# owkin/PyDESeq2

Measured on AMD Instinct MI355X. Metric: genes/sec end-to-end deseq2() (size factors->dispersion->IRLS->Wald), higher is better.
Workload: dtype f64

## Files before the change

### include/deseq_hip.h

```cpp
#ifndef DESEQ_HIP_H
#define DESEQ_HIP_H

#include <stddef.h>
#include <stdint.h>

#ifdef __cplusplus
extern "C" {
#endif

#define DSQ_ABI_VERSION 5
#define DSQ_MAX_P 128
#define DSQ_SHRINK_MAX_P 48
#define DSQ_BFGS_MAX_P 12

typedef struct dsq_ctx dsq_ctx;

enum dsq_status {
    DSQ_OK = 0,
    DSQ_ERR_HIP = -1,
    DSQ_ERR_ARG = -2,
    DSQ_ERR_RANGE = -3,
    DSQ_ERR_NOMEM = -4
};

// ... 138 lines not shown
                       int N, int G, int P, const double* d_alpha_hat, double min_disp, double max_disp,
                       double prior_disp_var, int cr_reg, int prior_reg, double* d_alpha, uint8_t* d_converged,
                       int32_t* d_nfev, double* d_nll_const, int const_mode, const dsq_cells* cells,
                       const double* d_coef, const double* d_sf, double min_mu);
int dsq_dev_alpha_mle3(dsq_ctx* ctx, const int32_t* d_y, const double* d_mu, int ldn, const double* d_Xt, int ldx,
                       int N, int G, int P, const double* d_alpha_hat, double min_disp, double max_disp,
                       double prior_disp_var, int cr_reg, int prior_reg, double* d_alpha, uint8_t* d_converged,
                       int32_t* d_nfev, double* d_nll_const, int const_mode, const dsq_cells* cells,
                       const double* d_coef, const double* d_sf, double min_mu, const int32_t* d_rows, int n_rows,
                       const int32_t* d_waves, int n_waves, const double* d_cell_mu);
typedef struct dsq_mix dsq_mix;
int dsq_mix_create(dsq_ctx* ctx, const double* design, int N, int P, dsq_mix** out);
void dsq_mix_destroy(dsq_mix* mix);
int dsq_mix_info(const dsq_mix* mix, int* n_slots, int* n_cells, int* n_continuous);
int dsq_mix_slots(const dsq_mix* mix, int32_t* h_slot_of);
int dsq_mix_bind(dsq_ctx* ctx, const uint16_t* d_ys, const uint8_t* d_big, const double* d_mu_slots);
int dsq_mix_bind2(dsq_ctx* ctx, const uint16_t* d_ys, const uint8_t* d_big, const double* d_mu_slots, int G);
int dsq_dev_mix_counts_to_slots(dsq_ctx* ctx, const int32_t* d_y, int ldn, int G, const dsq_mix* mix, uint16_t* d_ys,
                                uint8_t* d_big);
int dsq_dev_mix_mu_slots(dsq_ctx* ctx, const dsq_mix* mix, const double* d_beta, const double* d_sf, int G,
                         double* d_mu_slots);
int dsq_mix_takes_irls(const dsq_mix* mix, int full_rank);
int dsq_mix_launch_count(void);
int dsq_dev_alpha_mle4(dsq_ctx* ctx, const int32_t* d_y, const double* d_mu, int ldn, const double* d_Xt, int ldx,
                       int N, int G, int P, const double* d_alpha_hat, double min_disp, double max_disp,
                       double prior_disp_var, int cr_reg, int prior_reg, double* d_alpha, uint8_t* d_converged,
                       int32_t* d_nfev, double* d_nll_const, int const_mode, const dsq_cells* cells,
                       const double* d_coef, const double* d_sf, double min_mu, const int32_t* d_rows, int n_rows,
                       const int32_t* d_waves, int n_waves, const double* d_cell_mu, const dsq_mix* mix,
                       const double* d_beta);
int dsq_alpha_rows_eligible(int N, int P, int n_cells);
int dsq_alpha_needs_mu(int N, int P, int n_cells);
int dsq_dev_cell_mu(dsq_ctx* ctx, const double* d_beta, const dsq_cells* cells, int G, int P, double* d_cell_mu);
int dsq_dev_alpha_row_split(dsq_ctx* ctx, const int32_t* d_y, int ldn, int N, int G, int32_t* d_flags);
int dsq_dev_robust_disp(dsq_ctx* ctx, const int32_t* d_y, int ldn, const double* d_sf, const int32_t* d_cell_offsets,
                        const int32_t* d_cell_index, int n_cells, int whole, int max_cell, int N, int G,
                        double* d_robust_disp);
int dsq_dev_robust_disp2(dsq_ctx* ctx, const int32_t* d_y, int ldn, const double* d_sf, const int32_t* d_cell_offsets,
                         const int32_t* d_cell_index, int n_cells, int whole, int max_cell, int min_cell, int N, int G,
                         double* d_robust_disp);
int dsq_dev_lfc_fit(dsq_ctx* ctx, const int32_t* d_y, int ldn, const double* d_sf, const double* d_Xt,
                    const double* d_pinvXt, int ldx, int N, int G, int P, int full_rank, const double* d_disp,
                    double min_mu, double beta_tol, double min_beta, double max_beta, int maxiter, double* d_beta,
                    double* d_mu, double* d_hat, uint8_t* d_converged, int32_t* d_iters, const dsq_cells* cells,
                    const double* d_robust_disp, const uint8_t* d_flags, double cutoff, double* d_cooks,
                    uint8_t* d_any_all, uint8_t* d_any_use, uint8_t* d_any_use_nr, uint8_t* d_few_above,
// ... 144 lines not shown
```

### pydeseq2_amd/_lib.py

```python
from __future__ import annotations

import ctypes as C
import os

import numpy as np

_HERE = os.path.dirname(os.path.abspath(__file__))
LIB_PATH = os.environ.get("DSQ_LIB", os.path.join(_HERE, "libdeseq_hip.so"))

DSQ_MAX_P = 128
DSQ_SHRINK_MAX_P = 48
_DEBUG = bool(os.environ.get("DSQ_DEBUG"))
SAMPLE_MAJOR, GENE_MAJOR = 0, 1
I32, I64 = 0, 1
ALT = {None: 0, "greaterAbs": 1, "lessAbs": 2, "greater": 3, "less": 4}

c_void_p, c_int, c_double, c_size_t = C.c_void_p, C.c_int, C.c_double, C.c_size_t
_vp = c_void_p
HOOK_FN = C.CFUNCTYPE(None, c_void_p)


class DsqCells(C.Structure):

    _fields_ = [("d_cell_of", C.c_void_p), ("d_Xc", C.c_void_p), ("d_XX", C.c_void_p), ("n_cells", C.c_int)]
# ... 105 lines not shown
          c_double, c_int, _vp, _vp, _vp)
    proto("dsq_dev_lfc_shrink", _vp, _vp, c_int, _vp, _vp, c_int, c_int, c_int, c_int, _vp, c_double, c_double,
          c_int, _vp, _vp, _vp)
    proto("dsq_dev_lfc_shrink2", _vp, _vp, c_int, _vp, _vp, c_int, c_int, c_int, c_int, _vp, c_double, c_double,
          c_int, _vp, _vp, _vp, _vp)
    proto("dsq_dev_lfc_shrink3", _vp, _vp, c_int, _vp, _vp, c_int, c_int, c_int, c_int, _vp, c_double, c_double,
          c_int, _vp, _vp, _vp, _vp, c_int)
    proto("dsq_dev_padj_prepare", _vp, _vp, _vp, c_int, c_double, _vp, _vp, _vp, _vp, C.POINTER(c_int))
    proto("dsq_dev_padj_finish", _vp, _vp, _vp, _vp, c_int, c_int, c_int, _vp)
    proto("dsq_d2d", _vp, _vp, _vp, c_size_t)
    cells_p = C.POINTER(DsqCells)
    proto("dsq_dev_mom_lin_coef", _vp, _vp, c_int, _vp, _vp, _vp, c_int, c_int, c_int, c_int, c_double, c_double,
          c_double, _vp, _vp, _vp, _vp)
    proto("dsq_dev_alpha_mle2", _vp, _vp, _vp, c_int, _vp, c_int, c_int, c_int, c_int, _vp, c_double, c_double,
          c_double, c_int, c_int, _vp, _vp, _vp, _vp, c_int, cells_p, _vp, _vp, c_double)
    proto("dsq_dev_alpha_mle3", _vp, _vp, _vp, c_int, _vp, c_int, c_int, c_int, c_int, _vp, c_double, c_double,
          c_double, c_int, c_int, _vp, _vp, _vp, _vp, c_int, cells_p, _vp, _vp, c_double, _vp, c_int, _vp, c_int, _vp)
    proto("dsq_dev_alpha_mle4", _vp, _vp, _vp, c_int, _vp, c_int, c_int, c_int, c_int, _vp, c_double, c_double,
          c_double, c_int, c_int, _vp, _vp, _vp, _vp, c_int, cells_p, _vp, _vp, c_double, _vp, c_int, _vp, c_int, _vp,
          _vp, _vp)
    proto("dsq_mix_create", _vp, _vp, c_int, c_int, C.POINTER(_vp))
    proto("dsq_mix_destroy", _vp, res=None)
    proto("dsq_mix_launch_count")
    proto("dsq_mix_slots", _vp, _vp)
    proto("dsq_mix_takes_irls", _vp, c_int)
    proto("dsq_mix_info", _vp, C.POINTER(c_int), C.POINTER(c_int), C.POINTER(c_int))
    proto("dsq_alpha_rows_eligible", c_int, c_int, c_int)
    proto("dsq_alpha_needs_mu", c_int, c_int, c_int)
    proto("dsq_dev_cell_mu", _vp, _vp, cells_p, c_int, c_int, _vp)
    proto("dsq_dev_alpha_row_split", _vp, _vp, c_int, c_int, c_int, _vp)
    proto("dsq_dev_robust_disp", _vp, _vp, c_int, _vp, _vp, _vp, c_int, c_int, c_int, c_int, c_int, _vp)
    proto("dsq_dev_robust_disp2", _vp, _vp, c_int, _vp, _vp, _vp, c_int, c_int, c_int, c_int, c_int, c_int, _vp)
    proto("dsq_dev_lfc_fit", _vp, _vp, c_int, _vp, _vp, _vp, c_int, c_int, c_int, c_int, c_int, _vp, c_double,
          c_double, c_double, c_double, c_int, _vp, _vp, _vp, _vp, _vp, cells_p, _vp, _vp, c_double, _vp, _vp, _vp,
          _vp, _vp, _vp, _vp, c_double, c_int, _vp, _vp, _vp)
    proto("dsq_dev_lfc_fit2", _vp, _vp, c_int, _vp, _vp, _vp, c_int, c_int, c_int, c_int, c_int, _vp, c_double,
          c_double, c_double, c_double, c_int, _vp, _vp, _vp, _vp, _vp, cells_p, _vp, _vp, c_double, _vp, _vp, _vp,
          _vp, _vp, _vp, _vp, c_double, c_int, _vp, _vp, _vp, _vp, c_int)
    proto("dsq_dev_irls_layers", _vp, _vp, c_int, _vp, _vp, c_int, c_int, c_int, c_int, _vp, _vp, c_double, _vp, _vp)
    proto("dsq_side_begin", _vp)
    proto("dsq_side_end", _vp)
    proto("dsq_side_wait", _vp)
    proto("dsq_side_abort", _vp)
    proto("dsq_set_deferred", _vp, c_int)
    proto("dsq_lfc_fork_begin", _vp)
    proto("dsq_lfc_fork_end", _vp)
# ... 42 lines not shown
    return lib


EXPORTS = [
    "dsq_create", "dsq_destroy", "dsq_last_error", "dsq_device_info", "dsq_sync", "dsq_debug_pending_error", "dsq_timer_start",
    "dsq_timer_stop", "dsq_last_alpha_kernel", "dsq_malloc", "dsq_free", "dsq_memset", "dsq_h2d", "dsq_d2h", "dsq_h2d_2d",
    "dsq_d2h_2d", "dsq_inf_lin_reg_mu", "dsq_inf_irls", "dsq_inf_alpha_mle", "dsq_inf_wald_test",
    "dsq_inf_fit_rough_dispersions", "dsq_inf_fit_moments_dispersions", "dsq_dev_trend_loss_grad", "dsq_dev_trend_fit", "dsq_dev_prior_mad",
    "dsq_dev_counts_to_gene_major", "dsq_dev_f64_to_gene_major", "dsq_dev_logmeans",
    "dsq_dev_size_factors", "dsq_dev_mom", "dsq_dev_lin_mu", "dsq_dev_alpha_mle", "dsq_dev_irls",
    "dsq_dev_cooks", "dsq_dev_replace_outliers", "dsq_dev_wald", "dsq_dev_gather_rows_f64",
    "dsq_dev_gather_rows_i32", "dsq_comm_unique_id", "dsq_comm_init", "dsq_comm_destroy",
    "dsq_comm_allreduce_sum", "dsq_comm_allgather", "dsq_dev_sf_keys", "dsq_dev_sf_count", "dsq_dev_sf_init",
    "dsq_dev_sf_hist", "dsq_dev_sf_pick", "dsq_dev_sf_finish", "dsq_dev_trend_eval", "dsq_dev_trend_prior", "dsq_dev_select_dispersions",
    "dsq_dev_scatter_rows_f64", "dsq_d2d", "dsq_dev_mom_lin_mu", "dsq_dev_sf_keys_compact", "dsq_prior_mad_work_doubles", "dsq_size_factors_work_doubles", "dsq_dev_mom_raw", "dsq_dev_nll_const", "dsq_dev_nll_scaled", "dsq_dev_logmeans_poscounts", "dsq_dev_vst", "dsq_inf_lfc_shrink_nbinom_glm", "dsq_dev_lfc_shrink", "dsq_dev_lfc_shrink2", "dsq_dev_lfc_shrink3", "dsq_dev_padj_prepare", "dsq_dev_padj_finish", "dsq_host_alloc", "dsq_host_free", "dsq_d2h_async", "dsq_h2d_async",
    "dsq_dev_size_factors_new", "dsq_dev_mom_lin_coef", "dsq_dev_alpha_mle2", "dsq_dev_robust_disp", "dsq_dev_robust_disp2", "dsq_dev_lfc_fit", "dsq_dev_lfc_fit2", "dsq_dev_irls_layers",
    "dsq_side_begin", "dsq_side_end", "dsq_side_wait", "dsq_side_abort", "dsq_set_deferred", "dsq_irls_order_hint", "dsq_set_alpha_hook", "dsq_dev_alpha_mle3", "dsq_dev_alpha_mle4", "dsq_mix_create", "dsq_mix_destroy", "dsq_mix_info", "dsq_mix_slots", "dsq_mix_takes_irls", "dsq_dev_replace_outliers2", "dsq_mix_launch_count", "dsq_alpha_rows_eligible", "dsq_alpha_needs_mu", "dsq_dev_cell_mu", "dsq_dev_alpha_row_split",
    "dsq_upload_counts_i32", "dsq_inf_dispersion_trend_gamma_glm", "dsq_inf_grid_fit_alpha", "dsq_inf_grid_fit_beta",
    "dsq_inf_irls2", "dsq_inf_alpha_mle2", "dsq_inf_lfc_shrink_nbinom_glm2", "dsq_inf_fit_moments_dispersions2",
    "dsq_abi_version", "dsq_plugin_cache_config", "dsq_plugin_cache_clear", "dsq_plugin_cache_stats",
    "dsq_plugin_digest_host", "dsq_comm_info", "dsq_host_sync_count", "dsq_dev_pack2", "dsq_dev_unzip2",
    "dsq_mix_bind", "dsq_mix_bind2", "dsq_dev_mix_counts_to_slots", "dsq_dev_mix_mu_slots",
    "dsq_lfc_fork_begin", "dsq_lfc_fork_end", "dsq_lfc_set_part", "dsq_lfc_takes_parts", "dsq_dev_select_dispersions_part", "dsq_lfc_prepare", "dsq_alpha_set_late_flags",
    "dsq_dev_lrt", "dsq_dev_chisq_sf", "dsq_dev_wald_multi", "dsq_dev_rlog",
]


def ptr(a):
    if a is None:
        return None
    if isinstance(a, np.ndarray):
        return a.ctypes.data
    return a


class Context:

    def __init__(self, device: int = 0):
        self.lib = load()
        h = _vp()
        rc = self.lib.dsq_create(int(device), C.byref(h))
        if rc != 0 or not h.value:
            raise DsqError(
                f"dsq_create(device={device}) failed (rc={rc}): no usable MI355X / HIP runtime. "
                "pydeseq2_amd runs on the GPU only."
            )
        self.h = h
# ... 176 lines not shown
```

### pydeseq2_amd/csrc/dsq_capi_dev.hip

```cpp
#include "dsq_capi_internal.h"

extern "C" {

int dsq_dev_counts_to_gene_major(dsq_ctx* ctx, const void* d_src, int count_type, int layout, int N, int G,
                                 int32_t* d_dst, int ldn, int* h_bad) {
    DSQ_CHECK_ARG(ldn >= N, "ldn < N");
    int* d_bad = (int*)ctx->d_scratch;
    DSQ_HIP(hipMemsetAsync(d_bad, 0, sizeof(int), ctx->stream));
    DSQ_HIP(dsq::launch_transpose_counts(ctx->stream, d_src, count_type, layout, N, G, d_dst, ldn, d_bad));
    if (h_bad) {
        DSQ_HIP(hipMemcpyAsync(h_bad, d_bad, sizeof(int), hipMemcpyDeviceToHost, ctx->stream));
        DSQ_HIP(hipStreamSynchronize(ctx->stream));
    }
    return DSQ_OK;
}

int dsq_dev_f64_to_gene_major(dsq_ctx* ctx, const double* d_src, int layout, int N, int G, double* d_dst,
                              int ldn) {
    DSQ_HIP(dsq::launch_transpose_f64(ctx->stream, d_src, layout, N, G, d_dst, ldn));
    return DSQ_OK;
}

int dsq_dev_logmeans(dsq_ctx* ctx, const int32_t* d_y, int ldn, int N, int G, double* d_logmeans,
                     uint8_t* d_nonzero) {
// ... 355 lines not shown
    const int rc = dsq_mix_bind(ctx, d_ys, d_big, d_mu_slots);
    ctx->bind_G = (rc == DSQ_OK && G > 0) ? G : 0;
    return rc;
}
int dsq_dev_mix_counts_to_slots(dsq_ctx* ctx, const int32_t* d_y, int ldn, int G, const dsq_mix* mix, uint16_t* d_ys,
                                uint8_t* d_big) {
    DSQ_CHECK_ARG(mix != nullptr && d_y != nullptr && d_ys != nullptr && d_big != nullptr, "null argument");
    DSQ_HIP(dsq::launch_mix_counts_to_slots(ctx->stream, d_y, ldn, mix->d, G, d_ys, d_big));
    return DSQ_OK;
}
int dsq_dev_mix_mu_slots(dsq_ctx* ctx, const dsq_mix* mix, const double* d_beta, const double* d_sf, int G,
                         double* d_mu_slots) {
    DSQ_CHECK_ARG(mix != nullptr && d_beta != nullptr && d_sf != nullptr && d_mu_slots != nullptr, "null argument");
    DSQ_HIP(dsq::launch_mix_mu_slots(ctx->stream, d_beta, d_sf, mix->d, G, d_mu_slots));
    return DSQ_OK;
}

int dsq_mix_takes_irls(const dsq_mix* mix, int full_rank) {
    return (mix != nullptr && dsq::irls_takes_mix(&mix->d, full_rank)) ? 1 : 0;
}

int dsq_mix_launch_count(void) { return dsq::alpha_mix_launches(); }

int dsq_mix_info(const dsq_mix* mix, int* n_slots, int* n_cells, int* n_continuous) {
    if (mix == nullptr) return DSQ_ERR_ARG;
    if (n_slots) *n_slots = mix->d.Ns;
    if (n_cells) *n_cells = mix->d.C;
    if (n_continuous) *n_continuous = mix->d.Q;
    return DSQ_OK;
}

int dsq_alpha_needs_mu(int N, int P, int n_cells) { return dsq::alpha_needs_mu(N, P, n_cells) ? 1 : 0; }

int dsq_alpha_rows_eligible(int N, int P, int n_cells) {
    if (dsq::alpha_rows_eligible(N, P, n_cells, true, 1)) return 1;
    return dsq::alpha_rowsc_tail(N, P, n_cells) > 0 ? 2 : 0;
}

int dsq_dev_cell_mu(dsq_ctx* ctx, const double* d_beta, const dsq_cells* cells, int G, int P, double* d_cell_mu) {
    DSQ_CHECK_ARG(P >= 1 && P <= 12 && cells != nullptr && cells->n_cells > 0, "cells / P out of range");
    DSQ_HIP(dsq::launch_cell_mu(ctx->stream, d_beta, cells->d_Xc, cells->n_cells, G, P, d_cell_mu));
    return DSQ_OK;
}

int dsq_dev_alpha_row_split(dsq_ctx* ctx, const int32_t* d_y, int ldn, int N, int G, int32_t* d_flags) {
    DSQ_HIP(dsq::launch_count_big(ctx->stream, d_y, ldn, N, G, d_flags));
// ... 464 lines not shown
```

### pydeseq2_amd/csrc/dsq_irls.h

```cpp
#pragma once
#include "dsq_alpha.h"
#include "dsq_bfgs.h"
#include "dsq_lbfgsb.h"
#include "dsq_linalg.h"
#include "dsq_stats.h"
#include "dsq_wave.h"

#ifndef DSQ_IRLS_UNROLL
#define DSQ_IRLS_UNROLL 2
#endif
#define DSQ_PRAGMA_(x) _Pragma(#x)
#define DSQ_PRAGMA(x) DSQ_PRAGMA_(x)
#define DSQ_UNROLL2 DSQ_PRAGMA(unroll DSQ_IRLS_UNROLL)
#ifndef DSQ_IRLS_ROW_U
#define DSQ_IRLS_ROW_U 4
#endif

namespace dsq {

constexpr int kIrlsRowU = DSQ_IRLS_ROW_U;

struct LfcEpilogue {
    const uint8_t* flags = nullptr;
    double robust_disp = 0.0, cutoff = 0.0;
// ... 172 lines not shown
#pragma unroll
        for (int k = 0; k < NR; ++k)
            if (Wv::lane() + k * Wv::W < P) Wk.ent[T + Wv::lane() + k * Wv::W] = vr[k];
    }
    Wv::sync();
    if constexpr (LOADM) {
#pragma unroll
        for (int k = 0; k < T; ++k) M[k] = Wk.ent[k];
#pragma unroll
        for (int j = 0; j < P; ++j) r[j] = Wk.ent[T + j];
        Wv::sync();
    }
    S = Wv::sum(s);
}

template <int CS>
DSQ_HD double cell_select(int cell, const double (&v)[CS]) {
    double r = v[0];
#pragma unroll
    for (int c = 1; c < CS; ++c) r = (cell == c) ? v[c] : r;
    return r;
}

template <class Wv, int P, int CS>
DSQ_HD void irls_sweep_cs(const IrlsArgs& A, const double (&beta)[P], double a, double& S,
                          double (&M)[Tri<P>::N], double (&r)[P], double (&e_c)[CS]) {
    constexpr int T = Tri<P>::N;
    const CellDesign& D = *A.cells;
    const auto Xc_ = DSQ_AS_LDS(double, D.Xc);
    const auto XX_ = DSQ_AS_LDS(double, D.XX);
    double eta_c[CS], sw[CS], swz[CS];
#pragma unroll
    for (int c = 0; c < CS; ++c) {
        double eta = 0.0;
        if (c < D.C) {
#pragma unroll
            for (int j = 0; j < P; ++j) eta += Xc_[c * P + j] * beta[j];
        }
        eta_c[c] = Wv::uniform(eta);
        e_c[c] = Wv::uniform(exp(eta));
        sw[c] = 0.0;
        swz[c] = 0.0;
    }
    double s = 0.0;
    const double lmin = log(A.min_mu);
    DSQ_PHASE(3);
// ... 81 lines not shown
            const double h = w * cell_select<CS>(cell, q_c);
            if (H_out != nullptr) H_out[n] = h;
            if (want_cooks) {
                const double ck = acc.add(n, (double)A.y[n], mu_raw, h, E->flags[n]);
                if (E->cooks_row != nullptr) E->cooks_row[n] = ck;
            }
        }
        if (want_wald) {
            double wu = w;
            if (!have_w || Wv::any(!(mu_raw >= A.min_mu))) wu = mu_raw * frcp_g(1.0 + mu_raw * A.disp);
#pragma unroll
            for (int c = 0; c < CS; ++c) swu[c] += (cell == c) ? wu : 0.0;
        }
    }
    if (want_cooks) E->cooks = acc.finish(A.y, A.N);
    if (want_wald) {
        double Mw[T];
#pragma unroll
        for (int k = 0; k < T; ++k) Mw[k] = 0.0;
#pragma unroll
        for (int c = 0; c < CS; ++c) {
            if (c < D.C) {
                const double sc = Wv::sum(swu[c]);
#pragma unroll
                for (int k = 0; k < T; ++k) Mw[k] += XX_[c * T + k] * sc;
            }
        }
        E->wald = wald_from_M<P>(Mw, beta, E->ridge, E->contrast, E->lfc_null, E->alt);
    }
}

struct IrlsOut {
    int converged;
    int iters;
    int fallback;
};

template <class Wv, int P>
DSQ_HD void irls_init(const IrlsArgs& A, double a, double (&b0)[P], double& cst) {
#pragma unroll
    for (int j = 0; j < P; ++j) b0[j] = 0.0;
    double lga, dga_unused, tab_dl, tab_dd;
    lgamma_digamma<false, true>(a, lga, dga_unused);
    lgamma_digamma_diff<Wv, false>(Wv::lane(), a, lga, 0.0, tab_dl, tab_dd);
    double c = 0.0;
    for (int base = 0; base < A.N; base += Wv::W) {
// ... 267 lines not shown
            }
        }
    }
    for (; n < A.N; n += Wv::W) {
        const int cell = D.cell_of[n];
        const double wu = sample(n, cell, A.sf[n], Wk.tab[1][cell], Wk.acc[0][cell],
                                 want_cooks ? (double)A.y[n] : 0.0, want_cooks ? E->flags[n] : 0);
        if (want_wald) Wv::cell_add(&Wk.acc[1][cell], wu);
    }
    if (want_cooks) E->cooks = acc.finish(A.y, A.N);
    if (want_wald) {
        Wv::sync();
        for (int e = Wv::lane(); e < T; e += Wv::W) {
            Wk.ent[e] = cell_dot<T>(XX_ + e, Wk.acc[1], D.C);
        }
        Wv::sync();
        double Mw[T];
#pragma unroll
        for (int k = 0; k < T; ++k) Mw[k] = Wk.ent[k];
        E->wald = wald_from_M<P>(Mw, beta, E->ridge, E->contrast, E->lfc_null, E->alt);
    }
}

template <class Wv, int P, int CELL = 0>
DSQ_HD IrlsOut irls_gene(const IrlsArgs& A, double (&beta)[P], double* mu_out, double* H_out,
                         LfcEpilogue* E = nullptr) {
    constexpr int T = Tri<P>::N;
    IrlsOut out;
    out.converged = 1; out.iters = 0; out.fallback = 0;
    const double a = 1.0 / A.disp;
    double cst;
    DSQ_PHASE(1);
    if constexpr (CELL == 1 && Wv::W == 16) {
        if (A.pinvc != nullptr) irls_init_cell<Wv, P>(A, a, beta, cst);
        else irls_init<Wv, P>(A, a, beta, cst);
    } else {
        irls_init<Wv, P>(A, a, beta, cst);
    }
    const double nlogterm = A.N * a * log(A.disp);
    double M[T], r[P], S;
    constexpr int CS = CELL == 3 ? 2 : kSmallCells;
    double e_c[CS];
    constexpr bool kRowSolve = CELL == 1 && Wv::W == 16;
    auto sweep = [&]() {
        DSQ_PHASE(2);
        if constexpr (CELL == 1) irls_sweep_cell<Wv, P, !kRowSolve>(A, beta, a, S, M, r);
        else if constexpr (CELL >= 2) irls_sweep_cs<Wv, P, CS>(A, beta, a, S, M, r, e_c);
        else irls_sweep<Wv, P>(A, beta, a, S, M, r);
        DSQ_PHASE(5);
    };
    sweep();
    double dev = 1000.0, ratio = 1.0;
    int i = 0;
    while (ratio > A.beta_tol) {
        double bh[P];
        if constexpr (kRowSolve) {
            typedef DSQ_LDS_STRUCT(CellWork<P>) LdsWork;
            DSQ_PHASE(7);
            row_chol_solve<Wv, P>(((LdsWork*)A.cell_ws)->ent, 1e-6, bh);
            Wv::sync();
        } else {
            double Hm[T];
#pragma unroll
            for (int k = 0; k < T; ++k) Hm[k] = M[k];
#pragma unroll
            for (int j = 0; j < P; ++j) Hm[tri(j, j)] += 1e-6;
            DSQ_PHASE(7);
            chol<P>(Hm);
            DSQ_PHASE(8);
#pragma unroll
            for (int j = 0; j < P; ++j) bh[j] = r[j];
            chol_solve<P>(Hm, bh);
        }
        DSQ_PHASE(5);
        i += 1;
        bool bad = (i >= A.maxiter);
#pragma unroll
        for (int j = 0; j < P; ++j) bad = bad || (fabs(bh[j]) > A.max_beta);
        if (bad) {
            out.fallback = 1; out.converged = 0; out.iters = i;
            return out;
        }
#pragma unroll
        for (int j = 0; j < P; ++j) beta[j] = bh[j];
        sweep();
        const double old = dev;
        dev = -2.0 * (nlogterm - cst + S);
        ratio = fabs(dev - old) / (fabs(dev) + 0.1);
    }
    out.iters = i;
    DSQ_PHASE(6);
    if constexpr (kRowSolve) {
        typedef DSQ_LDS_STRUCT(CellWork<P>) LdsWork;
        LdsWork& Wk = *(LdsWork*)A.cell_ws;
#pragma unroll
        for (int k = 0; k < T; ++k) M[k] = Wk.ent[k];
        Wv::sync();
    }
    if constexpr (CELL == 1) irls_finish_cell<Wv, P>(A, beta, M, mu_out, H_out, E);
    else if constexpr (CELL >= 2) irls_finish_cs<Wv, P, CS>(A, beta, M, e_c, mu_out, H_out, E);
    else irls_finish<Wv, P>(A, beta, M, mu_out, H_out, E);
    return out;
}

template <int P>
struct IrlsRescueWork {
    union {
        LbfgsbWork<P> lb;
        BfgsWork<P> bf;
    };
    double x[P], l[P], u[P];
    int nbd[P];
};

template <class Wv>
DSQ_HD void grid_fit_beta2(const IrlsArgs& A, double a, double cst, double (&beta)[2],
                           int grid_length = 60) {
    auto loss = [&](double bx, double by) {
        double s = 0.0;
        DSQ_UNROLL2
    for (int n = Wv::lane(); n < A.N; n += Wv::W) {
            const double yv = (double)A.y[n];
            const double eta = A.Xt[n] * bx + A.Xt[A.ldx + n] * by;
// ... 91 lines not shown
```

### pydeseq2_amd/csrc/dsq_k_irls.hip

```cpp
#include <type_traits>

#include "dsq_dispatch.h"
#include "dsq_irls.h"
#include "dsq_launch.h"

namespace dsq {

#if defined(DSQ_PHASE_TIMING)
__device__ unsigned long long g_phase_total_irls[16];
#endif

#ifndef DSQ_IRLS_WAVES_P2
#define DSQ_IRLS_WAVES_P2 4
#endif
constexpr int irls_min_waves(int p) { return p <= 2 ? DSQ_IRLS_WAVES_P2 : (p <= 5 ? 1 : 2); }

template <int P, int CELL>
__global__ __launch_bounds__(kBlock, CELL == 1 ? cell_min_waves(P) : irls_min_waves(P)) void k_irls(const int32_t* __restrict__ y, int ldn,
                                                 const double* __restrict__ sf, const double* __restrict__ lsf,
                                                 const double* __restrict__ Xt,
                                                 const double* __restrict__ pinvXt, int ldx, int N,
                                                 int G, int full_rank, const double* __restrict__ disp,
                                                 double min_mu, double beta_tol, double min_beta,
                                                 double max_beta, int maxiter, double* __restrict__ beta,
                                                 double* __restrict__ mu, double* __restrict__ hat,
                                                 uint8_t* __restrict__ conv, int32_t* __restrict__ iters,
                                                 int32_t* __restrict__ fb_count,
                                                 int32_t* __restrict__ fb_list, IrlsExtras ex, int stage) {
    __shared__ typename std::conditional<CELL == 1, CellWork<P>, char>::type cellw[kWavesPerBlock];
    extern __shared__ __attribute__((aligned(16))) double irls_lds[];
    const int w = threadIdx.x >> 6;
    const int g = blockIdx.x * kWavesPerBlock + w;
    if (ex.part != nullptr) {
        bool any = false;
#pragma unroll
        for (int k = 0; k < kWavesPerBlock; ++k) {
            const int gk = blockIdx.x * kWavesPerBlock + k;
            any = any || (gk < G && ex.part[gk] == (uint8_t)ex.part_want);
        }
        if (!any) return;
// ... 26 lines not shown
        sf = s_sf;
        if (lsf != nullptr) lsf = s_lsf;
        if (CELL) ex.cells.cell_of = s_cell;
        yrow = s_y;
    }
    __syncthreads();
    if (g >= G) return;
    if (ex.part != nullptr && ex.part[g] != (uint8_t)ex.part_want) return;
#if defined(DSQ_PHASE_TIMING)
    if ((threadIdx.x & 63) == 0) {
        for (int k = 0; k < kPhases; ++k) g_ph_acc[w][k] = 0;
        g_ph_last[w] = clock64();
        g_ph_cur[w] = 0;
    }
#endif
    IrlsArgs A;
    A.y = yrow; A.sf = sf; A.lsf = lsf; A.Xt = Xt; A.pinvXt = pinvXt; A.ldx = ldx; A.N = N;
    A.disp = disp[g]; A.min_mu = min_mu; A.beta_tol = beta_tol; A.min_beta = min_beta;
    A.max_beta = max_beta; A.maxiter = maxiter; A.full_rank = full_rank != 0;
    if (CELL) { A.cells = &ex.cells; A.cell_ws = CELL == 1 ? (void*)&cellw[w] : nullptr; }
    LfcEpilogue E;
    epilogue_begin(E, ex, g, ldn);
    double b[P];
    const IrlsOut o = irls_gene<DeviceWave, P, CELL>(A, b, mu ? mu + (size_t)g * ldn : nullptr,
                                                     hat ? hat + (size_t)g * ldn : nullptr, &E);
    if ((threadIdx.x & 63) == 0) {
#pragma unroll
        for (int j = 0; j < P; ++j) beta[(size_t)g * P + j] = b[j];
        conv[g] = (uint8_t)o.converged;
        if (iters != nullptr) iters[g] = o.iters;
        if (o.fallback) fb_list[atomicAdd(fb_count, 1)] = g;
        else epilogue_store(E, ex, g);
    }
#if defined(DSQ_PHASE_TIMING)
    DSQ_PHASE(0);
    if ((threadIdx.x & 63) == 0)
        for (int k = 0; k < kPhases; ++k) atomicAdd(&g_phase_total_irls[k], (unsigned long long)g_ph_acc[w][k]);
#endif
}

constexpr int kRowGenes = kBlock / 16;
template <int P>
__global__ __launch_bounds__(kBlock, 2) void k_irls_row(const int32_t* __restrict__ y, int ldn,
                                                        const double* __restrict__ sf, const double* __restrict__ lsf,
                                                        const double* __restrict__ Xt,
                                                        const double* __restrict__ pinvXt, int ldx, int N, int G,
                                                        int full_rank, const double* __restrict__ disp, double min_mu,
                                                        double beta_tol, double min_beta, double max_beta, int maxiter,
// ... 249 lines not shown
                                          Xt, ldx, N, G, disp, beta, min_mu, mu, hat))
    return hipGetLastError();
}

constexpr int kRowMinP = 3;
static bool row_wave_enabled() {
    static const bool v = getenv("DSQ_NO_ROW_WAVE") == nullptr;
    return v;
}
static int row_min_p() {
    static const int v = getenv("DSQ_ROW_MIN_P") ? atoi(getenv("DSQ_ROW_MIN_P")) : 5;
    return v;
}
static size_t row_lds_bytes(int C, int P, int N) {
    const int npad = (N + 15) & ~15;
    return (size_t)C * (P * (P + 1) / 2 + 2 * P) * sizeof(double) + (size_t)npad * 20 + (size_t)kMaxCells * 4;
}

static int irls_row_min_genes() {
    const char* e = getenv("DSQ_IRLS_ROW_MIN_G");
    return e ? atoi(e) : 1024;
}

bool irls_takes_parts(int N, int P_, int n_cells, const MixDesign* mix, int full_rank) {
    (void)N;
    if (mix != nullptr && irls_takes_mix(mix, full_rank)) return true;
    return !(P_ > DSQ_REG_MAX_P || (P_ >= wide_min_p() && (n_cells == 0 || wide_with_cells())));
}

bool irls_takes_rows(int N, int P_, int n_cells) {
    if (P_ > DSQ_REG_MAX_P || (P_ >= wide_min_p() && (n_cells == 0 || wide_with_cells()))) return false;
    return n_cells > kSmallCells && P_ >= kRowMinP && P_ >= row_min_p() && row_wave_enabled() &&
           row_lds_bytes(n_cells, P_, N) <= 40 * 1024;
}

#define DSQ_MIXI_DECL(Q_)                                                                                             \
    bool irls_mix_fits_q##Q_(int Ns, int P);                                                                          \
    void irls_mix_grid_q##Q_(int Ns, int P, int G, int* blocks, int* nw);                                             \
    hipError_t launch_irls_mix_q##Q_(hipStream_t, const int32_t*, int, const uint16_t*, const uint8_t*, const MixDesign&, \
                                     const double*, int, int32_t*, const double*, double, double, double, int, double*, \
                                     double*, double*, uint8_t*, int32_t*, int32_t*, int32_t*, const IrlsExtras&, void*, \
                                     size_t);
DSQ_MIXI_DECL(1)
DSQ_MIXI_DECL(2)
DSQ_MIXI_DECL(3)
#undef DSQ_MIXI_DECL
// ... 38 lines not shown
                       const double* Xt,
                       const double* pinvXt, int ldx, int N, int G, int P_, int full_rank,
                       const double* disp, double min_mu, double beta_tol, double min_beta,
                       double max_beta, int maxiter, double* beta, double* mu, double* hat,
                       uint8_t* conv, int32_t* iters, int32_t* fb_count, int32_t* fb_list,
                       const IrlsExtras* extras) {
    if (G <= 0) return hipSuccess;
    IrlsExtras ex{};
    if (extras != nullptr) ex = *extras;
    if (ex.mix != nullptr && ex.mix_work != nullptr && ex.mix_queue != nullptr && ex.mix_ys != nullptr &&
        ex.mix_big != nullptr && irls_takes_mix(ex.mix, full_rank))
        return launch_irls_mix(st, y, ldn, *ex.mix, sf, G, ex.mix_queue, disp, min_mu, beta_tol, max_beta, maxiter, beta,
                               mu, hat, conv, iters, fb_count, fb_list, ex, ex.mix_work, ex.mix_work_bytes);
    if (P_ > DSQ_REG_MAX_P || (P_ >= wide_min_p() && (ex.cells.C == 0 || wide_with_cells()))) {
        if (ex.cells.C > 0 && ex.cells.C <= kSmallCells) ex.cells = CellDesign{};
        return launch_wide_irls(st, y, ldn, sf, lsf, Xt, pinvXt, ldx, N, G, P_, full_rank, disp, min_mu, beta_tol,
                                min_beta, max_beta, maxiter, beta, mu, hat, conv, iters, fb_count, fb_list, &ex);
    }
    const dim3 grid(genes_to_blocks(G)), block(kBlock);
    const int npad = (N + 15) & ~15;
    const size_t stage_bytes = (size_t)npad * (16 + 4 + 4 * kWavesPerBlock);
    static const bool allow_stage = getenv("DSQ_IRLS_NO_STAGE") == nullptr;
    if (ex.cells.C > 0 && ex.cells.C <= kSmallCells && P_ <= 4) {
        DSQ_DISPATCH_P(P_, {
            if constexpr (P <= 4) {
                const size_t tables = (size_t)ex.cells.C * (Tri<P>::N + P) * sizeof(double);
                const int stage = allow_stage && tables + stage_bytes <= 48 * 1024;
                if (ex.cells.C <= 2 && P <= 2)
                    hipLaunchKernelGGL((k_irls<(P <= 2 ? P : 1), 3>), grid, block, tables + (stage ? stage_bytes : 0),
                                       st, y, ldn, sf, lsf, Xt, pinvXt, ldx, N, G, full_rank, disp, min_mu, beta_tol,
                                       min_beta, max_beta, maxiter, beta, mu, hat, conv, iters, fb_count, fb_list, ex,
                                       stage);
                else
                    hipLaunchKernelGGL((k_irls<P, 2>), grid, block, tables + (stage ? stage_bytes : 0), st, y, ldn,
                                       sf, lsf, Xt, pinvXt, ldx, N, G, full_rank, disp, min_mu, beta_tol, min_beta,
                                       max_beta, maxiter, beta, mu, hat, conv, iters, fb_count, fb_list, ex, stage);
            }
        })
    } else if (irls_takes_rows(N, P_, ex.cells.C) && G >= irls_row_min_genes()) {
        const dim3 grid_r((G + kRowGenes - 1) / kRowGenes);
        DSQ_DISPATCH_P(P_, {
            if constexpr (P >= kRowMinP)
                hipLaunchKernelGGL((k_irls_row<P>), grid_r, block, row_lds_bytes(ex.cells.C, P, N), st, y, ldn, sf, lsf,
                                   Xt, pinvXt, ldx, N, G, full_rank, disp, min_mu, beta_tol, min_beta, max_beta, maxiter,
                                   beta, mu, hat, conv, iters, fb_count, fb_list, ex);
        })
    } else if (ex.cells.C > kSmallCells && P_ >= 3) {
        DSQ_DISPATCH_P(P_, {
            if constexpr (P >= 3) {
                const size_t tables = (size_t)ex.cells.C * (Tri<P>::N + P) * sizeof(double);
                const int stage = allow_stage && tables + stage_bytes <= 48 * 1024;
                hipLaunchKernelGGL((k_irls<P, 1>), grid, block, tables + (stage ? stage_bytes : 0), st, y, ldn, sf,
                                   lsf, Xt, pinvXt, ldx, N, G, full_rank, disp, min_mu, beta_tol, min_beta, max_beta,
                                   maxiter, beta, mu, hat, conv, iters, fb_count, fb_list, ex, stage);
            }
        })
    } else {
        const int stage = allow_stage && stage_bytes <= 48 * 1024;
        DSQ_DISPATCH_P(P_, hipLaunchKernelGGL((k_irls<P, 0>), grid, block, stage ? stage_bytes : 0, st, y, ldn, sf,
// ... 68 lines not shown
```

### pydeseq2_amd/csrc/dsq_launch.h

```cpp
#pragma once
#include <hip/hip_runtime.h>

#include <cstdint>

#include "../../include/deseq_hip.h"
#include "dsq_irls.h"
#include "dsq_linalg.h"
#include "dsq_mix.h"

namespace dsq {

constexpr int kWavesPerBlock = 4;
constexpr int kBlock = 64 * kWavesPerBlock;

inline int genes_to_blocks(int G) { return (G + kWavesPerBlock - 1) / kWavesPerBlock; }

inline int current_device_cus() {
    static int cache[64] = {0};
    int dev = 0;
    if (hipGetDevice(&dev) != hipSuccess) return 0;
    if (dev >= 0 && dev < 64 && cache[dev] > 0) return cache[dev];
    hipDeviceProp_t prop;
    if (hipGetDeviceProperties(&prop, dev) != hipSuccess) return 0;
    if (dev >= 0 && dev < 64) cache[dev] = prop.multiProcessorCount;
// ... 74 lines not shown
size_t alpha_resume_bytes(int G);
constexpr int kRowTail = 512;
bool alpha_rows_eligible(int N, int P, int n_cells, bool has_coef, int cr_reg);
hipError_t launch_alpha_rows(hipStream_t st, const int32_t* y, int ldn, int N, const int32_t* list, int n_list,
                             int32_t* queue, const double* coef, const double* sf, const CellDesign& cells, int P,
                             double min_mu, const double* alpha_hat, double min_disp, double max_disp, double prior_var,
                             int cr_reg, int prior_reg, double* alpha, uint8_t* conv, int32_t* nfev, int32_t* grid_count,
                             int32_t* grid_list, double* nll_const, int const_mode, int eval_cap, void* park_state,
                             int32_t* park_count, int32_t* park_list);
hipError_t launch_count_big(hipStream_t st, const int32_t* y, int ldn, int N, int G, int32_t* out);
int alpha_rowsc_tail(int N, int P, int n_cells);
hipError_t launch_alpha_rows_c(hipStream_t st, const int32_t* y, int ldn, int N, const int32_t* list, int n_list,
                               int32_t* queue, const double* coef, const double* cell_mu, const double* sf,
                               const CellDesign& cells, int P, double min_mu, const double* alpha_hat, double min_disp,
                               double max_disp, double prior_var, int prior_reg, double* alpha, uint8_t* conv,
                               int32_t* nfev, int32_t* grid_count, int32_t* grid_list, double* nll_const,
                               int const_mode, int eval_cap, void* park_state, int32_t* park_count,
                               int32_t* park_list);
hipError_t launch_cell_mu(hipStream_t st, const double* beta, const double* Xc, int C, int G, int P, double* cell_mu);
hipError_t launch_mu_from_cells(hipStream_t st, const double* cell_mu, int C, const double* sf, const int32_t* cell_of,
                                int N, const int32_t* list, int n_list, double* dst, int ldn, int32_t* idx_out,
                                const int32_t* n_dev = nullptr);
bool alpha_mix_enabled();
int alpha_mix_launches();
bool alpha_mix_fits(const MixDesign& D);
hipError_t launch_alpha_mix(hipStream_t st, const uint16_t* ys, const double* mu_s, const MixDesign& D, const int32_t* list,
                            int n_list, const int32_t* n_dev, int32_t* queue, const double* alpha_hat, double min_disp,
                            double max_disp, double prior_var, int prior_reg, double* alpha, uint8_t* conv, int32_t* nfev,
                            int32_t* grid_count, int32_t* grid_list, double* nll_const, int const_mode, int eval_cap,
                            int resume, void* park_state, int32_t* park_count, int32_t* park_list);
hipError_t launch_mu_from_beta(hipStream_t st, const double* beta, const double* sf, const double* Xt, int ldx, int N,
                               int P, const int32_t* list, int n_list, double* dst, int ldn, int32_t* idx_out,
                               const int32_t* n_dev = nullptr);
bool alpha_wg_eligible(int N);
hipError_t launch_alpha_wg(hipStream_t st, const int32_t* y, int ldn, int N, const int32_t* list, const int32_t* n_dev,
                           int n_cap, const double* coef, const double* sf, const CellDesign& cells, int P,
                           double min_mu, const double* alpha_hat, double prior_var, int prior_reg, double* alpha,
                           uint8_t* conv, int32_t* nfev, int32_t* grid_count, int32_t* grid_list,
                           const double* nll_const, const void* park_state);
hipError_t launch_alpha_bfgs(hipStream_t st, const int32_t* y, const double* mu, int ldn, const double* Xt, int ldx,
                             int N, int G, int P, const double* alpha_hat, double min_disp, double max_disp,
                             double prior_var, int cr_reg, int prior_reg, double* alpha, uint8_t* conv,
                             int32_t* nfev, int32_t* grid_count, int32_t* grid_list);
hipError_t launch_alpha(hipStream_t st, const int32_t* y, const double* mu, int ldn, const double* Xt,
                        int ldx, int N, int G, int P, const double* alpha_hat, double min_disp,
                        double max_disp, double prior_var, int cr_reg, int prior_reg, double* alpha,
// ... 205 lines not shown
```

### pydeseq2_amd/csrc/dsq_math.h

```cpp
#pragma once
#include <cmath>
#include <cstdint>
#include <cstring>

#include "dsq_exp_table.h"
#include "dsq_log_table.h"

#if defined(__HIPCC__)
#include <hip/hip_runtime.h>
#define DSQ_HD __host__ __device__ __forceinline__
#define DSQ_D __device__ __forceinline__
#else
#define DSQ_HD inline
#define DSQ_D inline
#endif

#if defined(DSQ_PHASE_TIMING) && defined(__HIPCC__)
namespace dsq {
constexpr int kPhases = 12;
__shared__ long long g_ph_acc[4][kPhases];
__shared__ long long g_ph_last[4];
__shared__ int g_ph_cur[4];
__device__ __forceinline__ void phase_mark(int k) {
    __builtin_amdgcn_sched_barrier(0);
    if ((threadIdx.x & 63) == 0) {
        const int w = threadIdx.x >> 6;
        const long long t = clock64();
        g_ph_acc[w][g_ph_cur[w]] += t - g_ph_last[w];
        g_ph_last[w] = t;
        g_ph_cur[w] = k;
    }
    __builtin_amdgcn_sched_barrier(0);
}
}
#define DSQ_PHASE(k) ::dsq::phase_mark(k)
#else
#define DSQ_PHASE(k) ((void)0)
#endif

#if defined(__HIP_DEVICE_COMPILE__)
#define DSQ_NO_SPECULATE asm volatile("")
#else
#define DSQ_NO_SPECULATE ((void)0)
#endif

namespace dsq {

DSQ_HD double flog(double x);
DSQ_HD double flog_t(double x);
DSQ_HD double flog1p(double u);
DSQ_HD double frcp(double x);
DSQ_HD double frcp_g(double x);
DSQ_HD double frsq(double x);

constexpr double kHalfLog2Pi = 0.91893853320467274178032973640562;
constexpr double kEps = 2.220446049250313e-16;

DSQ_HD double stirling_tail(double rz) {
    const double r2 = rz * rz;
    double s = 6.4102564102564102564e-3;
    s = s * r2 - 1.9175269175269175269e-3;
    s = s * r2 + 8.4175084175084175084e-4;
    s = s * r2 - 5.9523809523809523810e-4;
    s = s * r2 + 7.9365079365079365079e-4;
    s = s * r2 - 2.7777777777777777778e-3;
    s = s * r2 + 8.3333333333333333333e-2;
    return s * rz;
}

// ... 263 lines not shown
```

Baseline: 10.78 million.

## Add current-cell walk accumulation to small-cell IRLS sweep and finish

Replaces the generic per-sample cell-indexed accumulation in the small-cell IRLS path with a 'current cell' walk. Each lane keeps scalar accumulators for the active cell and flushes them into per-cell arrays only when the wave sees a cell change, which targets the per-sample select/scatter work over all CS cells. It also drops the likelihood sum on the initial sweep, since it is not needed there. The old path stays reachable through the DSQ_CELL_WALK=generic environment variable, with launch counters added. A rounding barrier is added to keep the accumulation order the same as before, at the cost of extra branching when samples are not grouped by cell.

```diff
diff --git a/include/deseq_hip.h b/include/deseq_hip.h
--- a/include/deseq_hip.h
+++ b/include/deseq_hip.h
@@ -184,6 +184,7 @@
                          double* d_mu_slots);
 int dsq_mix_takes_irls(const dsq_mix* mix, int full_rank);
 int dsq_mix_launch_count(void);
+int dsq_cell_walk_launches(int generic);
 int dsq_dev_alpha_mle4(dsq_ctx* ctx, const int32_t* d_y, const double* d_mu, int ldn, const double* d_Xt, int ldx,
                        int N, int G, int P, const double* d_alpha_hat, double min_disp, double max_disp,
                        double prior_disp_var, int cr_reg, int prior_reg, double* d_alpha, uint8_t* d_converged,
diff --git a/pydeseq2_amd/_lib.py b/pydeseq2_amd/_lib.py
--- a/pydeseq2_amd/_lib.py
+++ b/pydeseq2_amd/_lib.py
@@ -151,6 +151,7 @@
     proto("dsq_mix_create", _vp, _vp, c_int, c_int, C.POINTER(_vp))
     proto("dsq_mix_destroy", _vp, res=None)
     proto("dsq_mix_launch_count")
+    proto("dsq_cell_walk_launches", c_int)
     proto("dsq_mix_slots", _vp, _vp)
     proto("dsq_mix_takes_irls", _vp, c_int)
     proto("dsq_mix_info", _vp, C.POINTER(c_int), C.POINTER(c_int), C.POINTER(c_int))
@@ -239,7 +240,7 @@
     "dsq_plugin_digest_host", "dsq_comm_info", "dsq_host_sync_count", "dsq_dev_pack2", "dsq_dev_unzip2",
     "dsq_mix_bind", "dsq_mix_bind2", "dsq_dev_mix_counts_to_slots", "dsq_dev_mix_mu_slots",
     "dsq_lfc_fork_begin", "dsq_lfc_fork_end", "dsq_lfc_set_part", "dsq_lfc_takes_parts", "dsq_dev_select_dispersions_part", "dsq_lfc_prepare", "dsq_alpha_set_late_flags",
-    "dsq_dev_lrt", "dsq_dev_chisq_sf", "dsq_dev_wald_multi", "dsq_dev_rlog",
+    "dsq_dev_lrt", "dsq_dev_chisq_sf", "dsq_dev_wald_multi", "dsq_dev_rlog", "dsq_cell_walk_launches",
 ]
 
 
diff --git a/pydeseq2_amd/csrc/dsq_capi_dev.hip b/pydeseq2_amd/csrc/dsq_capi_dev.hip
--- a/pydeseq2_amd/csrc/dsq_capi_dev.hip
+++ b/pydeseq2_amd/csrc/dsq_capi_dev.hip
@@ -401,6 +401,8 @@
 
 int dsq_mix_launch_count(void) { return dsq::alpha_mix_launches(); }
 
+int dsq_cell_walk_launches(int generic) { return dsq::cell_walk_launches(generic); }
+
 int dsq_mix_info(const dsq_mix* mix, int* n_slots, int* n_cells, int* n_continuous) {
     if (mix == nullptr) return DSQ_ERR_ARG;
     if (n_slots) *n_slots = mix->d.Ns;
diff --git a/pydeseq2_amd/csrc/dsq_irls.h b/pydeseq2_amd/csrc/dsq_irls.h
--- a/pydeseq2_amd/csrc/dsq_irls.h
+++ b/pydeseq2_amd/csrc/dsq_irls.h
@@ -1,4 +1,6 @@
 #pragma once
+#include <type_traits>
+
 #include "dsq_alpha.h"
 #include "dsq_bfgs.h"
 #include "dsq_lbfgsb.h"
@@ -218,6 +220,22 @@
     return r;
 }
 
+template <int CS>
+DSQ_HD void cell_put(int cell, double (&v)[CS], double x) {
+#pragma unroll
+    for (int c = 0; c < CS; ++c) v[c] = (cell == c) ? x : v[c];
+}
+
+template <int CS, int NA>
+DSQ_HD void cell_walk_switch(int& cur, int cell, double (&sums)[NA][CS], double (&acc)[NA]) {
+#pragma unroll
+    for (int k = 0; k < NA; ++k) {
+        cell_put<CS>(cur, sums[k], acc[k]);
+        acc[k] = cell_select<CS>(cell, sums[k]);
+    }
+    cur = cell;
+}
+
 template <class Wv, int P, int CS>
 DSQ_HD void irls_sweep_cs(const IrlsArgs& A, const double (&beta)[P], double a, double& S,
                           double (&M)[Tri<P>::N], double (&r)[P], double (&e_c)[CS]) {
@@ -345,6 +363,173 @@
         for (int c = 0; c < CS; ++c) {
             if (c < D.C) {
                 const double sc = Wv::sum(swu[c]);
+#pragma unroll
+                for (int k = 0; k < T; ++k) Mw[k] += XX_[c * T + k] * sc;
+            }
+        }
+        E->wald = wald_from_M<P>(Mw, beta, E->ridge, E->contrast, E->lfc_null, E->alt);
+    }
+}
+
+template <class Wv, int P, int CS, bool WANT_S>
+DSQ_HD void irls_sweep_cur(const IrlsArgs& A, const double (&beta)[P], double a, double& S,
+                           double (&M)[Tri<P>::N], double (&r)[P], double (&e_c)[CS]) {
+    constexpr int T = Tri<P>::N;
+    const CellDesign& D = *A.cells;
+    const auto Xc_ = DSQ_AS_LDS(double, D.Xc);
+    const auto XX_ = DSQ_AS_LDS(double, D.XX);
+    double eta_c[CS], sums[2][CS];
+#pragma unroll
+    for (int c = 0; c < CS; ++c) {
+        double eta = 0.0;
+        if (c < D.C) {
+#pragma unroll
+            for (int j = 0; j < P; ++j) eta += Xc_[c * P + j] * beta[j];
+        }
+        eta_c[c] = Wv::uniform(eta);
+        e_c[c] = Wv::uniform(exp(eta));
+        sums[0][c] = 0.0;
+        sums[1][c] = 0.0;
+    }
+    double s = 0.0;
+    const double lmin = log(A.min_mu);
+    int cur = 0;
+    double eta_cur = eta_c[0], e_cur = e_c[0], acc[2] = {0.0, 0.0};
+    DSQ_PHASE(3);
+    for (int n = Wv::lane(); n < A.N; n += Wv::W) {
+        const double yv = (double)A.y[n];
+        const double sfn = A.sf[n];
+        const int cell = D.cell_of[n];
+        if (Wv::any(cell != cur)) {
+            cell_walk_switch<CS, 2>(cur, cell, sums, acc);
+            eta_cur = cell_select<CS>(cell, eta_c);
+            e_cur = cell_select<CS>(cell, e_c);
+        }
+        const double mu_raw = rounded(sfn * e_cur);
+        const bool clamped = !(mu_raw > A.min_mu);
+        const double lsfn = (A.lsf != nullptr) ? A.lsf[n] : flog(sfn);
+        double w, wz;
+        if (Wv::any(clamped)) {
+            const double mu = clamped ? A.min_mu : mu_raw;
+            if constexpr (WANT_S) {
+                const double lmu = clamped ? lmin : eta_cur + lsfn;
+                s += (yv + a) * flog_t(a + mu) - yv * lmu;
+            }
+            const double rd = frcp(1.0 + mu * A.disp);
+            w = mu * rd;
+            wz = (mu * (clamped ? lmin - lsfn : eta_cur) + (yv - mu)) * rd;
+        } else {
+            const double mu = mu_raw;
+            if constexpr (WANT_S) {
+                const double lmu = eta_cur + lsfn;
+                s += (yv + a) * flog_t(a + mu) - yv * lmu;
+            }
+            const double rd = frcp(1.0 + mu * A.disp);
+            w = mu * rd;
+            wz = (mu * eta_cur + (yv - mu)) * rd;
+        }
+        acc[0] += rounded(w);
+        acc[1] += rounded(wz);
+    }
+    cell_put<CS>(cur, sums[0], acc[0]);
+    cell_put<CS>(cur, sums[1], acc[1]);
+    DSQ_PHASE(4);
+    {
+        constexpr int NS = WANT_S ? 1 : 0;
+        double v[NS + 2 * CS];
+        if constexpr (WANT_S) v[0] = s;
+#pragma unroll
+        for (int c = 0; c < CS; ++c) { v[NS + c] = sums[0][c]; v[NS + CS + c] = sums[1][c]; }
+        Wv::template sum_n<NS + 2 * CS>(v);
+        S = WANT_S ? v[0] : 0.0;
+#pragma unroll
+        for (int c = 0; c < CS; ++c) { sums[0][c] = v[NS + c]; sums[1][c] = v[NS + CS + c]; }
+    }
+#pragma unroll
+    for (int k = 0; k < T; ++k) M[k] = 0.0;
+#pragma unroll
+    for (int j = 0; j < P; ++j) r[j] = 0.0;
+#pragma unroll
+    for (int c = 0; c < CS; ++c) {
+        if (c < D.C) {
+#pragma unroll
+            for (int k = 0; k < T; ++k) M[k] += XX_[c * T + k] * sums[0][c];
+#pragma unroll
+            for (int j = 0; j < P; ++j) r[j] += Xc_[c * P + j] * sums[1][c];
+        }
+    }
+}
+
+template <class Wv, int P, int CS>
+DSQ_HD void irls_finish_cur(const IrlsArgs& A, const double (&beta)[P], double (&M)[Tri<P>::N],
+                            const double (&e_c)[CS], double* mu_out, double* H_out, LfcEpilogue* E = nullptr) {
+    constexpr int T = Tri<P>::N;
+    const bool want_cooks = E != nullptr && E->flags != nullptr;
+    const bool want_wald = E != nullptr && E->ridge != nullptr;
+    if (mu_out == nullptr && H_out == nullptr && !want_cooks && !want_wald) return;
+    const CellDesign& D = *A.cells;
+    const auto Xc_ = DSQ_AS_LDS(double, D.Xc);
+    const auto XX_ = DSQ_AS_LDS(double, D.XX);
+    double q_c[CS], sums[1][CS];
+    {
+        double rinv[P];
+#pragma unroll
+        for (int j = 0; j < P; ++j) M[tri(j, j)] += 1e-6;
+        chol<P>(M);
+        chol_rinv<P>(M, rinv);
+#pragma unroll
+        for (int c = 0; c < CS; ++c) {
+            double q = 0.0;
+            if (c < D.C) {
+                double x[P];
+#pragma unroll
+                for (int j = 0; j < P; ++j) x[j] = Xc_[c * P + j];
+                q = chol_quad<P>(M, rinv, x);
+            }
+            q_c[c] = Wv::uniform(q);
+            sums[0][c] = 0.0;
+        }
+    }
+    CooksAcc<Wv> acc(Wv::uniform(want_cooks ? E->robust_disp : 0.0), Wv::uniform(want_cooks ? E->cutoff : 0.0), P);
+    int cur = 0;
+    double e_cur = e_c[0], q_cur = q_c[0], acc_wu[1] = {0.0};
+    for (int n = Wv::lane(); n < A.N; n += Wv::W) {
+        const int cell = D.cell_of[n];
+        if (Wv::any(cell != cur)) {
+            cell_walk_switch<CS, 1>(cur, cell, sums, acc_wu);
+            e_cur = cell_select<CS>(cell, e_c);
+            q_cur = cell_select<CS>(cell, q_c);
+        }
+        const double mu_raw = A.sf[n] * e_cur;
+        if (mu_out != nullptr) mu_out[n] = mu_raw;
+        double w = 0.0;
+        const bool have_w = H_out != nullptr || want_cooks;
+        if (have_w) {
+            const double mu = dmax(mu_raw, A.min_mu);
+            w = mu * frcp_g(1.0 + mu * A.disp);
+            const double h = w * q_cur;
+            if (H_out != nullptr) H_out[n] = h;
+            if (want_cooks) {
+                const double ck = acc.add(n, (double)A.y[n], mu_raw, h, E->flags[n]);
+                if (E->cooks_row != nullptr) E->cooks_row[n] = ck;
+            }
+        }
+        if (want_wald) {
+            double wu = w;
+            if (!have_w || Wv::any(!(mu_raw >= A.min_mu))) wu = mu_raw * frcp_g(1.0 + mu_raw * A.disp);
+            acc_wu[0] += rounded(wu);
+        }
+    }
+    cell_put<CS>(cur, sums[0], acc_wu[0]);
+    if (want_cooks) E->cooks = acc.finish(A.y, A.N);
+    if (want_wald) {
+        double Mw[T];
+#pragma unroll
+        for (int k = 0; k < T; ++k) Mw[k] = 0.0;
+#pragma unroll
+        for (int c = 0; c < CS; ++c) {
+            if (c < D.C) {
+                const double sc = Wv::sum(sums[0][c]);
 #pragma unroll
                 for (int k = 0; k < T; ++k) Mw[k] += XX_[c * T + k] * sc;
             }
@@ -658,7 +843,7 @@
     }
 }
 
-template <class Wv, int P, int CELL = 0>
+template <class Wv, int P, int CELL = 0, bool GENERIC_WALK = false>
 DSQ_HD IrlsOut irls_gene(const IrlsArgs& A, double (&beta)[P], double* mu_out, double* H_out,
                          LfcEpilogue* E = nullptr) {
     constexpr int T = Tri<P>::N;
@@ -678,14 +863,15 @@
     constexpr int CS = CELL == 3 ? 2 : kSmallCells;
     double e_c[CS];
     constexpr bool kRowSolve = CELL == 1 && Wv::W == 16;
-    auto sweep = [&]() {
+    auto sweep = [&](auto want_s) {
         DSQ_PHASE(2);
         if constexpr (CELL == 1) irls_sweep_cell<Wv, P, !kRowSolve>(A, beta, a, S, M, r);
-        else if constexpr (CELL >= 2) irls_sweep_cs<Wv, P, CS>(A, beta, a, S, M, r, e_c);
+        else if constexpr (CELL >= 2 && GENERIC_WALK) irls_sweep_cs<Wv, P, CS>(A, beta, a, S, M, r, e_c);
+        else if constexpr (CELL >= 2) irls_sweep_cur<Wv, P, CS, decltype(want_s)::value>(A, beta, a, S, M, r, e_c);
         else irls_sweep<Wv, P>(A, beta, a, S, M, r);
         DSQ_PHASE(5);
     };
-    sweep();
+    sweep(std::false_type{});
     double dev = 1000.0, ratio = 1.0;
     int i = 0;
     while (ratio > A.beta_tol) {
@@ -719,7 +905,7 @@
         }
 #pragma unroll
         for (int j = 0; j < P; ++j) beta[j] = bh[j];
-        sweep();
+        sweep(std::true_type{});
         const double old = dev;
         dev = -2.0 * (nlogterm - cst + S);
         ratio = fabs(dev - old) / (fabs(dev) + 0.1);
@@ -734,7 +920,8 @@
         Wv::sync();
     }
     if constexpr (CELL == 1) irls_finish_cell<Wv, P>(A, beta, M, mu_out, H_out, E);
-    else if constexpr (CELL >= 2) irls_finish_cs<Wv, P, CS>(A, beta, M, e_c, mu_out, H_out, E);
+    else if constexpr (CELL >= 2 && GENERIC_WALK) irls_finish_cs<Wv, P, CS>(A, beta, M, e_c, mu_out, H_out, E);
+    else if constexpr (CELL >= 2) irls_finish_cur<Wv, P, CS>(A, beta, M, e_c, mu_out, H_out, E);
     else irls_finish<Wv, P>(A, beta, M, mu_out, H_out, E);
     return out;
 }
diff --git a/pydeseq2_amd/csrc/dsq_k_irls.hip b/pydeseq2_amd/csrc/dsq_k_irls.hip
--- a/pydeseq2_amd/csrc/dsq_k_irls.hip
+++ b/pydeseq2_amd/csrc/dsq_k_irls.hip
@@ -1,3 +1,4 @@
+#include <atomic>
 #include <type_traits>
 
 #include "dsq_dispatch.h"
@@ -15,7 +16,7 @@
 #endif
 constexpr int irls_min_waves(int p) { return p <= 2 ? DSQ_IRLS_WAVES_P2 : (p <= 5 ? 1 : 2); }
 
-template <int P, int CELL>
+template <int P, int CELL, bool GENERIC_WALK = false>
 __global__ __launch_bounds__(kBlock, CELL == 1 ? cell_min_waves(P) : irls_min_waves(P)) void k_irls(const int32_t* __restrict__ y, int ldn,
                                                  const double* __restrict__ sf, const double* __restrict__ lsf,
                                                  const double* __restrict__ Xt,
@@ -88,8 +89,8 @@
     LfcEpilogue E;
     epilogue_begin(E, ex, g, ldn);
     double b[P];
-    const IrlsOut o = irls_gene<DeviceWave, P, CELL>(A, b, mu ? mu + (size_t)g * ldn : nullptr,
-                                                     hat ? hat + (size_t)g * ldn : nullptr, &E);
+    const IrlsOut o = irls_gene<DeviceWave, P, CELL, GENERIC_WALK>(A, b, mu ? mu + (size_t)g * ldn : nullptr,
+                                                                   hat ? hat + (size_t)g * ldn : nullptr, &E);
     if ((threadIdx.x & 63) == 0) {
 #pragma unroll
         for (int j = 0; j < P; ++j) beta[(size_t)g * P + j] = b[j];
@@ -385,6 +386,13 @@
     return e ? atoi(e) : 1024;
 }
 
+static bool cell_walk_generic() {
+    const char* e = getenv("DSQ_CELL_WALK");
+    return e != nullptr && strcmp(e, "generic") == 0;
+}
+static std::atomic<int> g_cell_walk_launches[2];
+int cell_walk_launches(int generic) { return g_cell_walk_launches[generic ? 1 : 0].load(std::memory_order_relaxed); }
+
 bool irls_takes_parts(int N, int P_, int n_cells, const MixDesign* mix, int full_rank) {
     (void)N;
     if (mix != nullptr && irls_takes_mix(mix, full_rank)) return true;
@@ -469,19 +477,19 @@
     const size_t stage_bytes = (size_t)npad * (16 + 4 + 4 * kWavesPerBlock);
     static const bool allow_stage = getenv("DSQ_IRLS_NO_STAGE") == nullptr;
     if (ex.cells.C > 0 && ex.cells.C <= kSmallCells && P_ <= 4) {
+        const bool generic_walk = cell_walk_generic();
+        g_cell_walk_launches[generic_walk ? 1 : 0].fetch_add(1, std::memory_order_relaxed);
         DSQ_DISPATCH_P(P_, {
             if constexpr (P <= 4) {
                 const size_t tables = (size_t)ex.cells.C * (Tri<P>::N + P) * sizeof(double);
                 const int stage = allow_stage && tables + stage_bytes <= 48 * 1024;
-                if (ex.cells.C <= 2 && P <= 2)
-                    hipLaunchKernelGGL((k_irls<(P <= 2 ? P : 1), 3>), grid, block, tables + (stage ? stage_bytes : 0),
-                                       st, y, ldn, sf, lsf, Xt, pinvXt, ldx, N, G, full_rank, disp, min_mu, beta_tol,
-                                       min_beta, max_beta, maxiter, beta, mu, hat, conv, iters, fb_count, fb_list, ex,
-                                       stage);
-                else
-                    hipLaunchKernelGGL((k_irls<P, 2>), grid, block, tables + (stage ? stage_bytes : 0), st, y, ldn,
-                                       sf, lsf, Xt, pinvXt, ldx, N, G, full_rank, disp, min_mu, beta_tol, min_beta,
-                                       max_beta, maxiter, beta, mu, hat, conv, iters, fb_count, fb_list, ex, stage);
+                constexpr int P2 = P <= 2 ? P : 1;
+                const bool two = ex.cells.C <= 2 && P <= 2;
+                auto kern = two ? (generic_walk ? k_irls<P2, 3, true> : k_irls<P2, 3, false>)
+                                : (generic_walk ? k_irls<P, 2, true> : k_irls<P, 2, false>);
+                hipLaunchKernelGGL(kern, grid, block, tables + (stage ? stage_bytes : 0), st, y, ldn, sf, lsf, Xt,
+                                   pinvXt, ldx, N, G, full_rank, disp, min_mu, beta_tol, min_beta, max_beta, maxiter,
+                                   beta, mu, hat, conv, iters, fb_count, fb_list, ex, stage);
             }
         })
     } else if (irls_takes_rows(N, P_, ex.cells.C) && G >= irls_row_min_genes()) {
diff --git a/pydeseq2_amd/csrc/dsq_launch.h b/pydeseq2_amd/csrc/dsq_launch.h
--- a/pydeseq2_amd/csrc/dsq_launch.h
+++ b/pydeseq2_amd/csrc/dsq_launch.h
@@ -120,6 +120,7 @@
                                 int N, const int32_t* list, int n_list, double* dst, int ldn, int32_t* idx_out,
                                 const int32_t* n_dev = nullptr);
 bool alpha_mix_enabled();
+int cell_walk_launches(int generic);
 int alpha_mix_launches();
 bool alpha_mix_fits(const MixDesign& D);
 hipError_t launch_alpha_mix(hipStream_t st, const uint16_t* ys, const double* mu_s, const MixDesign& D, const int32_t* list,
diff --git a/pydeseq2_amd/csrc/dsq_math.h b/pydeseq2_amd/csrc/dsq_math.h
--- a/pydeseq2_amd/csrc/dsq_math.h
+++ b/pydeseq2_amd/csrc/dsq_math.h
@@ -45,6 +45,13 @@
 #endif
 
 namespace dsq {
+
+DSQ_HD double rounded(double x) {
+#if defined(__HIP_DEVICE_COMPILE__)
+    asm("" : "+v"(x));
+#endif
+    return x;
+}
 
 DSQ_HD double flog(double x);
 DSQ_HD double flog_t(double x);
```

Measured after the change: 11.02 million, median of 6. 1.02x the previous value.
